# mxngjxa/lshrs

Measured on AMD Instinct MI355X. Metric: vectors/sec hashed (768-d, num_perm=256), higher is better.
Workload: dtype bf16x3 on the matrix cores + f32 replay of the host BLAS inside the proven window (bit-exact f32 sign result)

## Files before the change

lshrs_amd/csrc/sig_replay.hip:

```cpp
#include "lshrs_common.h"

using namespace lshrs;

namespace {
__device__ __forceinline__ void fix_chain_tile(const f32x4 (&p4)[2][4], const f32x4 (&x4)[2][4], float& acc, float& ss) {
#pragma unroll
  for (int sstep = 0; sstep < 16; ++sstep) {
    const int q = sstep >> 2, r = sstep & 3;
    acc = __builtin_fmaf(x4[0][q][r], p4[0][q][r], acc);
    acc = __builtin_fmaf(x4[1][q][r], p4[1][q][r], acc);
    ss = __builtin_fmaf(x4[0][q][r], x4[0][q][r], ss);
    ss = __builtin_fmaf(x4[1][q][r], x4[1][q][r], ss);
  }
}

__device__ __forceinline__ float blas_scalar_tail(float y, const float* __restrict__ pt, const float* __restrict__ xt, int m3,
                                                  int tail_model, bool count_ss, float* ss) {
  const float a0 = pt[0], x0 = xt[0];
  const float a1 = m3 > 1 ? pt[1] : 0.f, x1 = m3 > 1 ? xt[1] : 0.f;
  const float a2 = m3 > 2 ? pt[2] : 0.f, x2 = m3 > 2 ? xt[2] : 0.f;
  if (count_ss) *ss = __builtin_fmaf(x0, x0, __builtin_fmaf(x1, x1, __builtin_fmaf(x2, x2, *ss)));
  if (tail_model == 2) {
    float t = mul_then_add(0.f, a0, x0);
    if (m3 > 1) t = mul_then_add(t, a1, x1);
    if (m3 > 2) t = mul_then_add(t, a2, x2);
    return mul_then_add(y, t, 1.0f);
  }
  if (m3 == 1) return __builtin_fmaf(a0, x0, y);
  float t = __builtin_fmaf(a0, x0, mul_then_add(0.f, a1, x1));
  if (m3 > 2) t = __builtin_fmaf(a2, x2, t);
  return mul_then_add(y, t, 1.0f);
}

static_assert(LSHRS_SIG_COUNTERS + kFixParts * kFixGridG <= LSHRS_SIG_DEVICE_COUNTERS, "stage 2's per-workgroup slots must fit the counter block");
template <bool REPLAY, bool GENERAL = false, int SLAB = kFixSlabG, bool SAMEP = false>
__global__ __launch_bounds__(64) void sig_fix8_kernel(const FixArgs a) {
  static_assert(!SAMEP || (REPLAY && SLAB * 8 <= 64), "the shared hyperplane slab is one LDS-DMA of the wave");
  __shared__ __attribute__((aligned(16))) f32x4 xs[2][SLAB * 8 * kFixG];
  __shared__ __attribute__((aligned(16))) f32x4 ps[2][SAMEP ? 64 : SLAB * 8 * kFixG];
  const int lane = threadIdx.x, g = lane & (kFixG - 1), sub = lane >> 3;
  const int shh = sub >> 2, sq = sub & 3;
  const int64_t* __restrict__ list = SAMEP ? a.sorted_list : a.flag_list;
  const float* __restrict__ ylist = SAMEP ? a.sorted_y : a.flag_y;
  __shared__ int gstart[SAMEP ? kSortMaxCols + 1 : 1];
  const bool buckets = SAMEP && a.col_cap > 0;
  if (SAMEP && buckets) {
    constexpr int kPer = kSortMaxCols / 64;
    int mine[kPer], sum = 0;
    bool over = false;
#pragma unroll
    for (int i = 0; i < kPer; ++i) {
      const int c = lane * kPer + i;
      const int want = c < a.padcols ? a.col_count[c] : 0;
      over = over || want > a.col_cap;
      mine[i] = ((want < a.col_cap ? want : a.col_cap) + kFixG - 1) / kFixG;
      sum += mine[i];
    }
    int incl = sum;
#pragma unroll
    for (int off = 1; off < 64; off <<= 1) {
      const int v = __shfl_up(incl, off);
      if (lane >= off) incl += v;
    }
    int at = incl - sum;
#pragma unroll
    for (int i = 0; i < kPer; ++i) {
      gstart[lane * kPer + i] = at;
      at += mine[i];
    }
    if (lane == 63) gstart[kSortMaxCols] = at;
    if (blockIdx.x == 0 && __any(over) && lane == 0) *a.overflow = 1;
    __syncthreads();
  }
  const int cnt = !SAMEP ? min(*a.flag_count, a.flag_cap) : gstart[kSortMaxCols] * kFixG;
  const int fgroups = (cnt + kFixG - 1) / kFixG;
  const int groups = fgroups + (!SAMEP && REPLAY && a.audit_list != nullptr ? (a.audit_n + kFixG - 1) / kFixG : 0);
  const size_t ldp = (size_t)a.ktiles * kKTile;
  const int head = GENERAL ? (a.dim & 4) : 0;
  const int m3 = GENERAL ? (a.dim & 3) : 0;
  const int body = GENERAL ? a.dim - m3 - head : a.ktiles * kKTile;
  const int kt = GENERAL ? (body + kKTile - 1) / kKTile : a.ktiles;
  const int slabs = (kt + SLAB - 1) / SLAB;
  int n_ties = 0, n_flips = 0, n_aud = 0, n_abad = 0;
  float max_dev = 0.f, max_ratio = 0.f;
  struct Item { int64_t row; int col; bool live; const float* xg; const float* pg; const float* xrow; int e; bool audit; };
  auto fetch = [&](int grp) {
    Item it;
    it.audit = grp >= fgroups;
    int64_t item;
    bool inlist;
    if (SAMEP && buckets) {
      int lo = 0, hi = a.padcols - 1;
      while (lo < hi) {
        const int mid = (lo + hi + 1) >> 1;
        if (gstart[mid] <= grp) lo = mid; else hi = mid - 1;
      }
      const int off = (grp - gstart[lo]) * kFixG + g;
      const int have = min(a.col_count[lo], a.col_cap);
      inlist = off < have;
      it.e = lo * a.col_cap + (inlist ? off : 0);
      item = list[it.e];
      it.audit = (item & kAuditBit) != 0;
      item &= ~kAuditBit;
    } else if (!it.audit) {
      it.e = grp * kFixG + g;
      inlist = it.e < cnt;
      item = list[inlist ? it.e : grp * kFixG];
    } else {
      it.e = (grp - fgroups) * kFixG + g;
      item = it.e < a.audit_n ? a.audit_list[it.e] : -1;
      inlist = item >= 0;
      if (!inlist) item = 0;
    }
    it.row = entry_row(item);
    const int col_raw = entry_col(item);
    it.live = inlist && col_raw < a.padcols;
    it.col = col_raw < a.padcols ? col_raw : 0;
    it.xrow = a.X + it.row * a.ldx;
    it.xg = it.xrow + head + 16 * shh + 4 * sq;
    it.pg = a.prow + (size_t)it.col * ldp + head + 16 * shh + 4 * sq;
#ifdef LSHRS_AB_FIX_SAME_P
    {
      const int c0 = entry_col(a.flag_list[grp * kFixG < cnt ? grp * kFixG : 0]);
      it.pg = a.prow + (size_t)(c0 < a.padcols ? c0 : 0) * ldp + 16 * shh + 4 * sq;
    }
#endif
    return it;
  };
  auto issue = [&](const Item& it, int slab, int buf) {
#pragma unroll
    for (int i = 0; i < SLAB; ++i) {
      const int t = slab * SLAB + i < kt ? slab * SLAB + i : kt - 1;
#ifndef LSHRS_AB_FIX_NO_X
      const float* xsrc = it.xg + (size_t)t * kKTile;
      if (GENERAL && t * kKTile + 16 * shh + 4 * sq >= body) xsrc = it.xrow;
      __builtin_amdgcn_global_load_lds((const GLOBAL_AS void*)xsrc, (LDS_AS void*)(xs[buf] + i * 64), 16, 0, 0);
#endif
#ifndef LSHRS_AB_FIX_NO_P
      if (!SAMEP)
        __builtin_amdgcn_global_load_lds((const GLOBAL_AS void*)(it.pg + (size_t)t * kKTile), (LDS_AS void*)(ps[buf] + i * 64),
                                         16, 0, 0);
#endif
    }
    if (SAMEP) {
      const int ti = (lane >> 3) < SLAB ? (lane >> 3) : SLAB - 1;
      const int t = slab * SLAB + ti < kt ? slab * SLAB + ti : kt - 1;
      const float* psrc = a.prow + (size_t)it.col * ldp + head + (size_t)t * kKTile + 4 * (lane & 7);
      __builtin_amdgcn_global_load_lds((const GLOBAL_AS void*)psrc, (LDS_AS void*)ps[buf], 16, 0, 0);
    }
  };
  int grp = blockIdx.x;
  if (grp < groups) {
  Item cur = fetch(grp);
  issue(cur, 0, 0);
  int buf = 0;
  for (;;) {
    const int nxt_grp = grp + (int)gridDim.x;
    const bool has_next = nxt_grp < groups;
    Item nxt = cur;
    if (has_next) nxt = fetch(nxt_grp);
    const int64_t row = cur.row;
    const int col = cur.col, e = cur.e;
    const bool live = cur.live;
    const int word = col >> 5, c = col & 31;
    float acc = 0.f, ss = 0.f, pj = 0.f, ytot = 0.f;
    bool blocks_done = false;
    const int kind = GENERAL ? blas_row_kind(col % a.band_cols, a.rows_per_band) : 0;
    if (GENERAL && head != 0) {
      const int hl = kind == 1 ? (sub & 3) : sub;
      if (hl < 4) {
        const float hx = cur.xrow[hl];
        pj = a.prow[(size_t)col * ldp + hl] * hx;
        if (sub < 4) ss = hx * hx;
      }
    }
    for (int sl = 0; sl < slabs; ++sl) {
      const int tiles = kt - sl * SLAB < SLAB ? kt - sl * SLAB : SLAB;
      bool more = true;
      if (sl + 1 < slabs) issue(cur, sl + 1, buf ^ 1);
      else if (has_next) issue(nxt, 0, buf ^ 1);
      else more = false;
#if defined(LSHRS_AB_FIX_NO_X) || defined(LSHRS_AB_FIX_NO_P)
      if (more) wait_vmcnt<SLAB>();
#else
      if (more) wait_vmcnt<SAMEP ? SLAB + 1 : 2 * SLAB>();
#endif
      else asm volatile("s_waitcnt vmcnt(0)" ::: "memory");
      if (REPLAY) {
        const float* xf = reinterpret_cast<const float*>(xs[buf]);
        const float* pf = reinterpret_cast<const float*>(ps[buf]);
        if (!GENERAL) {
#pragma unroll 3
          for (int t = 0; t < tiles; ++t) {
#pragma unroll
            for (int m = 0; m < 4; ++m) {
              const int o = ((t * 8 + 2 * m + (sub >> 2)) * kFixG + g) * 4 + (sub & 3);
              const int op = SAMEP ? (t * 8 + 2 * m + (sub >> 2)) * 4 + (sub & 3) : o;
              const float xv = xf[o];
              pj = __builtin_fmaf(pf[op], xv, pj);
              ss = __builtin_fmaf(xv, xv, ss);
            }
          }
        } else {
          for (int t = 0; t < tiles; ++t) {
            const int kb0 = (sl * SLAB + t) * kKTile;
#pragma unroll
            for (int m = 0; m < 4; ++m) {
              const int o = ((t * 8 + 2 * m + (sub >> 2)) * kFixG + g) * 4 + (sub & 3);
              const int op = SAMEP ? (t * 8 + 2 * m + (sub >> 2)) * 4 + (sub & 3) : o;
              const bool in = kb0 + 8 * m + sub < body;
              const float xv = in ? xf[o] : 0.f, pv = in ? pf[op] : 0.f;
              ss = __builtin_fmaf(xv, xv, ss);
              if (kind == 1) {
                const int o0 = ((t * 8 + 2 * m) * kFixG + g) * 4 + (sub & 3), o1 = o0 + kFixG * 4;
                const int p0 = SAMEP ? (t * 8 + 2 * m) * 4 + (sub & 3) : o0, p1 = SAMEP ? p0 + 4 : o1;
                const int kl = kb0 + 8 * m + (sub & 3);
                pj = mul_then_add(pj, kl < body ? pf[p0] : 0.f, kl < body ? xf[o0] : 0.f);
                pj = mul_then_add(pj, kl + 4 < body ? pf[p1] : 0.f, kl + 4 < body ? xf[o1] : 0.f);
              } else if (kind == 2) {
                pj = mul_then_add(pj, pv, xv);
              } else {
                pj = __builtin_fmaf(pv, xv, pj);
              }
            }
            const int tile = sl * SLAB + t + 1;
            if ((tile % kBlasBlockTiles) == 0 && tile < kt) {
              const float sblk = blas_reduce(pj, kind, lane);
              ytot = blocks_done ? ytot + sblk : sblk;
              blocks_done = true;
              pj = 0.f;
            }
          }
        }
      } else {
#pragma unroll 2
        for (int t = 0; t < tiles; ++t) {
          f32x4 p4[2][4], x4[2][4];
#pragma unroll
          for (int hh = 0; hh < 2; ++hh)
#pragma unroll
            for (int q = 0; q < 4; ++q) {
              x4[hh][q] = xs[buf][(t * 8 + hh * 4 + q) * kFixG + g];
              p4[hh][q] = ps[buf][(t * 8 + hh * 4 + q) * kFixG + g];
            }
          fix_chain_tile(p4, x4, acc, ss);
        }
      }
      asm volatile("s_waitcnt lgkmcnt(0)" ::: "memory");
      buf ^= 1;
    }
    float yb = 0.f;
    if (REPLAY) {
      yb = blas_reduce(pj, kind, lane);
      if (GENERAL && blocks_done) yb = ytot + yb;
      if (GENERAL && m3 != 0)
        yb = blas_scalar_tail(yb, a.prow + (size_t)col * ldp + head + body, cur.xrow + head + body, m3, a.tail_model, sub == 0, &ss);
      float s2 = ss + __shfl(ss, (lane + 32) & 63);
      s2 += __shfl(s2, (lane + 8) & 63);
      ss = s2 + __shfl(s2, (lane + 16) & 63);
    }
    if (REPLAY && cur.audit) {
      if (sub == 0 && live) {
        const uint8_t kbyte = a.keys[row * (int64_t)a.row_bytes + (col >> 3)];
        ++n_aud;
        if ((yb > 0.f) != (((kbyte >> (col & 7)) & 1) != 0)) ++n_abad;
        const float y1 = (SAMEP && buckets) ? ylist[e] : a.audit_vals[2 * e];
        const float thr = (SAMEP && buckets) ? a.flag_thr[e] : a.audit_vals[2 * e + 1];
        if (thr > 0.f) {
          const float ratio = __builtin_fabsf(y1 - yb) / thr;
          if (ratio < __builtin_inff()) max_ratio = __builtin_fmaxf(max_ratio, ratio);
        }
      }
    } else if (sub == 0 && live) {
    uint8_t* kb = a.keys + row * (int64_t)a.row_bytes + (col >> 3);
    const uintptr_t addr = reinterpret_cast<uintptr_t>(kb);
    unsigned int* w32 = reinterpret_cast<unsigned int*>(addr & ~(uintptr_t)3);
    const unsigned int bitmask = 1u << (8 * (unsigned)(addr & 3) + (col & 7));
    bool want = acc > 0.f;
    const bool have = (*kb >> (col & 7)) & 1;
    if (REPLAY) {
      want = yb > 0.f;
      const float scale = sqrtf(ss) * a.norms[col];
      if (__builtin_fabsf(yb) < a.tau * sqrtf(ss) * a.tie_coef[col]) ++n_ties;
      if (want != have) ++n_flips;
      if (ylist != nullptr && scale > 0.f) {
        const float dev = __builtin_fabsf(ylist[e] - yb) / (scale * 0x1p-24f);
        if (dev < __builtin_inff()) max_dev = __builtin_fmaxf(max_dev, dev);
      }
    }
    if (want != have) {
      if (want) atomicOr(w32, bitmask);
      else atomicAnd(w32, ~bitmask);
    }
    if (!REPLAY && a.tie_list != nullptr) {
      const float thr = a.tau * sqrtf(ss) * a.tie_coef[col];
      if (__builtin_fabsf(acc) < thr) {
        const int slot = atomicAdd(a.tie_count, 1);
        if (slot < a.tie_cap) {
          a.tie_list[2 * (int64_t)slot] = (row + a.row_base) * 65536 + word;
          a.tie_list[2 * (int64_t)slot + 1] = (int64_t)(1u << c);
        }
      }
    }
    if (REPLAY && a.replay_y != nullptr) a.replay_y[e] = yb;
    }
    if (!has_next) break;
    cur = nxt;
    grp = nxt_grp;
  }
  }
  if (REPLAY) {
#pragma unroll
    for (int off = 1; off < 8; off <<= 1) {
      n_ties += __shfl_xor(n_ties, off);
      n_flips += __shfl_xor(n_flips, off);
      max_dev = __builtin_fmaxf(max_dev, __shfl_xor(max_dev, off));
      n_aud += __shfl_xor(n_aud, off);
      n_abad += __shfl_xor(n_abad, off);
      max_ratio = __builtin_fmaxf(max_ratio, __shfl_xor(max_ratio, off));
    }
    if (lane == 0) {
      int* p = a.partials + kFixParts * blockIdx.x;
      p[0] = a.count_ties ? n_ties : 0;
      p[1] = n_flips;
      p[2] = __float_as_int(max_dev);
      p[3] = n_aud;
      p[4] = n_abad;
      p[5] = __float_as_int(max_ratio);
    }
  }
}

__global__ void expand_ties_kernel(const int64_t* __restrict__ tie_list, const int* __restrict__ tie_count, int tie_cap,
                                   int padcols, int64_t* __restrict__ flag_list, int flag_cap, int* flag_count) {
  const int cnt = min(*tie_count, tie_cap);
  for (int e = blockIdx.x * blockDim.x + threadIdx.x; e < cnt; e += gridDim.x * blockDim.x) {
    const int64_t row = tie_list[2 * (int64_t)e] >> 16;
    const int word = (int)(tie_list[2 * (int64_t)e] & 0xFFFF);
    unsigned mask = (unsigned)tie_list[2 * (int64_t)e + 1];
    const int m = __popc(mask);
    if (m == 0) continue;
    int slot = atomicAdd(flag_count, m);
    while (mask != 0u) {
      const int c = __ffs(mask) - 1;
      mask &= mask - 1u;
      const int col = 32 * word + c;
      if (slot < flag_cap && col < padcols) flag_list[slot] = flag_entry(row, col);
      else if (slot < flag_cap) flag_list[slot] = flag_entry(row, (1 << kEntryColBits) - 1);
      ++slot;
    }
  }
}

__device__ __forceinline__ float mul_rounded(float a, float b) {
#pragma clang fp contract(off)
  return a * b;
}
__device__ __forceinline__ float add_rounded(float a, float b) {
#pragma clang fp contract(off)
  return a + b;
}
__device__ __forceinline__ float small_skx_dot(const float* __restrict__ a, const float* __restrict__ x, int n, int row, int rows) {
  auto p = [&](int k) { return mul_rounded(a[k], x[k]); };
  auto f = [&](int k, float s) { return __builtin_fmaf(a[k], x[k], s); };
  const int b16 = rows / 16 * 16, b8 = rows / 8 * 8;
  int rem = rows - b8, type;
  if (row < b16) type = 16;
  else if (row < b8) type = 8;
  else if (rem >= 4 && row < b8 + 4) type = 4;
  else {
    const int base = b8 + (rem >= 4 ? 4 : 0);
    rem -= rem >= 4 ? 4 : 0;
    type = (rem >= 2 && row < base + 2) ? 2 : 1;
  }
  auto seq = [&]() {
    float s = p(0);
    for (int k = 1; k < n; ++k) s = add_rounded(s, p(k));
    return s;
  };
  auto chain = [&]() {
    float s = p(0);
    for (int k = 1; k < n; ++k) s = f(k, s);
    return s;
  };
  switch (n) {
    case 1: return p(0);
    case 2: return type == 16 ? f(1, p(0)) : add_rounded(p(0), p(1));
    case 3:
      if (type >= 8) return f(2, f(1, p(0)));
      if (type == 2) return add_rounded(add_rounded(p(0), p(1)), p(2));
      return f(2, f(0, p(1)));
    case 4: return type == 1 ? seq() : add_rounded(add_rounded(p(0), p(1)), add_rounded(p(2), p(3)));
    case 5: return type >= 4 ? chain() : seq();
    case 6:
      if (type >= 8) return chain();
      if (type == 4) return add_rounded(add_rounded(p(0), f(1, p(2))), add_rounded(p(3), f(4, p(5))));
      return seq();
    case 7:
      if (type >= 8) return chain();
      if (type == 4) return add_rounded(add_rounded(f(0, p(1)), f(4, p(5))), add_rounded(f(2, p(3)), p(6)));
      return seq();
    default:
      if (type >= 4)
        return add_rounded(add_rounded(add_rounded(p(0), p(1)), add_rounded(p(2), p(3))), add_rounded(add_rounded(p(4), p(5)), add_rounded(p(6), p(7))));
      if (type == 2)
        return add_rounded(add_rounded(add_rounded(p(0), p(1)), add_rounded(p(4), p(5))), add_rounded(add_rounded(p(2), p(3)), add_rounded(p(6), p(7))));
      return add_rounded(add_rounded(add_rounded(add_rounded(p(0), p(4)), add_rounded(p(1), p(5))), add_rounded(p(2), p(6))), add_rounded(p(3), p(7)));
  }
}

__global__ __launch_bounds__(64) void sig_fixany_kernel(const FixArgs a) {
  const int lane = threadIdx.x, g = lane & (kFixG - 1), sub = lane >> 3;
  const int cnt = min(*a.flag_count, a.flag_cap);
  const int fgroups = (cnt + kFixG - 1) / kFixG;
  const int groups = fgroups + (a.audit_list != nullptr ? (a.audit_n + kFixG - 1) / kFixG : 0);
  const size_t ldp = (size_t)a.ktiles * kKTile;
  const int body = a.dim & ~3, m3 = a.dim & 3;
  int n_ties = 0, n_flips = 0, n_aud = 0, n_abad = 0;
  float max_dev = 0.f, max_ratio = 0.f;
  for (int grp = blockIdx.x; grp < groups; grp += gridDim.x) {
    const bool audit = grp >= fgroups;
    const int e = (audit ? grp - fgroups : grp) * kFixG + g;
    int64_t item;
    bool inlist;
    if (!audit) {
      inlist = e < cnt;
      item = a.flag_list[inlist ? e : grp * kFixG];
    } else {
      item = e < a.audit_n ? a.audit_list[e] : -1;
      inlist = item >= 0;
      if (!inlist) item = 0;
    }
    const int64_t row = entry_row(item);
    const int col_raw = entry_col(item);
    const bool live = inlist && col_raw < a.padcols;
    const int col = col_raw < a.padcols ? col_raw : 0;
    const float* __restrict__ xr = a.X + row * a.ldx;
    const float* __restrict__ pr = a.prow + (size_t)col * ldp;
    const int kind = blas_row_kind(col % a.band_cols, a.rows_per_band);
    float y = 0.f, ss = 0.f;
    if (a.tail_model == 3) {
      const int j = col % a.band_cols;
      y = j < a.rows_per_band ? small_skx_dot(pr, xr, a.dim, j, a.rows_per_band) : 0.f;
      if (sub == 0)
        for (int k = 0; k < a.dim; ++k) ss = __builtin_fmaf(xr[k], xr[k], ss);
    } else if (a.rows_per_band == 1) {
      const int n1 = a.dim & ~31;
      float kernel = 0.f;
      if (a.tail_model == 1) {
        const int n64 = n1 & ~63;
        float acc[8] = {0.f, 0.f, 0.f, 0.f, 0.f, 0.f, 0.f, 0.f};
        for (int k0 = 0; k0 < n64; k0 += 64)
#pragma unroll
          for (int j = 0; j < 8; ++j) {
            const float xv = xr[k0 + 8 * j + sub];
            acc[j] = __builtin_fmaf(pr[k0 + 8 * j + sub], xv, acc[j]);
            ss = __builtin_fmaf(xv, xv, ss);
          }
        float t[4];
#pragma unroll
        for (int u = 0; u < 4; ++u) t[u] = n64 > 0 ? acc[2 * u] + acc[2 * u + 1] : 0.f;
        if (n64 < n1) {
#pragma unroll
          for (int u = 0; u < 4; ++u) {
            const float xv = xr[n64 + 8 * u + sub];
            t[u] = __builtin_fmaf(pr[n64 + 8 * u + sub], xv, t[u]);
            ss = __builtin_fmaf(xv, xv, ss);
          }
        }
        const float v = ((t[0] + t[1]) + t[2]) + t[3];
        kernel = blas_reduce(v, 0, lane);
      } else {
        float acc[4] = {0.f, 0.f, 0.f, 0.f};
        for (int k0 = 0; k0 < n1; k0 += 32)
#pragma unroll
          for (int j = 0; j < 4; ++j) {
            const float xv = xr[k0 + 8 * j + sub];
            acc[j] = __builtin_fmaf(pr[k0 + 8 * j + sub], xv, acc[j]);
            ss = __builtin_fmaf(xv, xv, ss);
          }
        float sj[4];
#pragma unroll
// ... 23 lines not shown
      } else {
        const int head = kn & 4;
        if (head != 0 && sub < 4) {
          const float xv = xr[k0 + sub];
          pj = pr[k0 + sub] * xv;
          ss = __builtin_fmaf(xv, xv, ss);
        }
        for (int k = k0 + head + sub; k < k0 + kn; k += 8) {
          const float xv = xr[k];
          pj = kind == 0 ? __builtin_fmaf(pr[k], xv, pj) : mul_then_add(pj, pr[k], xv);
          ss = __builtin_fmaf(xv, xv, ss);
        }
      }
      const float sblk = blas_reduce(pj, kind, lane);
      y = k0 == 0 ? sblk : y + sblk;
    }
    if (m3 != 0 && a.rows_per_band != 1 && a.tail_model != 3)
      y = blas_scalar_tail(y, pr + body, xr + body, m3, a.tail_model, sub == 0, &ss);
    float s2 = ss + __shfl(ss, (lane + 32) & 63);
    s2 += __shfl(s2, (lane + 8) & 63);
    s2 += __shfl(s2, (lane + 16) & 63);
    if (sub == 0 && live && audit) {
      const uint8_t kbyte = a.keys[row * (int64_t)a.row_bytes + (col >> 3)];
      ++n_aud;
      if ((y > 0.f) != (((kbyte >> (col & 7)) & 1) != 0)) ++n_abad;
      const float thr = a.audit_vals[2 * e + 1];
      if (thr > 0.f) {
        const float ratio = __builtin_fabsf(a.audit_vals[2 * e] - y) / thr;
        if (ratio < __builtin_inff()) max_ratio = __builtin_fmaxf(max_ratio, ratio);
      }
    } else if (sub == 0 && live) {
      uint8_t* kb = a.keys + row * (int64_t)a.row_bytes + (col >> 3);
      const uintptr_t addr = reinterpret_cast<uintptr_t>(kb);
      unsigned int* w32 = reinterpret_cast<unsigned int*>(addr & ~(uintptr_t)3);
      const unsigned int bitmask = 1u << (8 * (unsigned)(addr & 3) + (col & 7));
      const bool want = y > 0.f;
      const bool have = (*kb >> (col & 7)) & 1;
      if (__builtin_fabsf(y) < a.tau * sqrtf(s2) * a.tie_coef[col]) ++n_ties;
      if (a.flag_y != nullptr) {
        const float scale = sqrtf(s2) * a.norms[col];
        if (scale > 0.f) {
          const float dev = __builtin_fabsf(a.flag_y[e] - y) / (scale * 0x1p-24f);
          if (dev < __builtin_inff()) max_dev = __builtin_fmaxf(max_dev, dev);
        }
      }
      if (want != have) {
        ++n_flips;
        if (want) atomicOr(w32, bitmask);
        else atomicAnd(w32, ~bitmask);
      }
      if (a.replay_y != nullptr) a.replay_y[e] = y;
    }
  }
#pragma unroll
  for (int off = 1; off < 8; off <<= 1) {
    n_ties += __shfl_xor(n_ties, off);
    n_flips += __shfl_xor(n_flips, off);
    max_dev = __builtin_fmaxf(max_dev, __shfl_xor(max_dev, off));
    n_aud += __shfl_xor(n_aud, off);
    n_abad += __shfl_xor(n_abad, off);
    max_ratio = __builtin_fmaxf(max_ratio, __shfl_xor(max_ratio, off));
  }
  if (lane == 0) {
    int* p = a.partials + kFixParts * blockIdx.x;
    p[0] = a.count_ties ? n_ties : 0;
    p[1] = n_flips;
    p[2] = __float_as_int(max_dev);
    p[3] = n_aud;
    p[4] = n_abad;
    p[5] = __float_as_int(max_ratio);
  }
}

constexpr int kExportThreads = 1024;
__global__ __launch_bounds__(kExportThreads) void export_counts_kernel(int* counters, int* host_counts, int nparts, int* zero = nullptr,
                                                                      int nzero = 0, int* done = nullptr, int epoch = 0) {
  __shared__ int fold[kExportThreads / 64][kFixParts];
  const int tid = threadIdx.x, lane = tid & 63, wave = tid >> 6;
  for (int i = tid; i < nzero; i += kExportThreads) zero[i] = 0;
  int* parts = counters + LSHRS_SIG_COUNTERS;
  int ties = 0, flips = 0, dev = 0, aud = 0, abad = 0, ratio = 0;
  for (int i = tid; i < nparts; i += kExportThreads) {
    int* q = parts + kFixParts * i;
    ties += q[0];
    flips += q[1];
    dev = max(dev, q[2]);
    aud += q[3];
    abad += q[4];
    ratio = max(ratio, q[5]);
    q[0] = q[1] = q[2] = q[3] = q[4] = q[5] = 0;
  }
#pragma unroll
  for (int off = 32; off >= 1; off >>= 1) {
    ties += __shfl_xor(ties, off);
    flips += __shfl_xor(flips, off);
    dev = max(dev, __shfl_xor(dev, off));
    aud += __shfl_xor(aud, off);
    abad += __shfl_xor(abad, off);
    ratio = max(ratio, __shfl_xor(ratio, off));
  }
  if (lane == 0) {
    fold[wave][0] = ties; fold[wave][1] = flips; fold[wave][2] = dev;
    fold[wave][3] = aud; fold[wave][4] = abad; fold[wave][5] = ratio;
  }
  __syncthreads();
  if (tid < LSHRS_SIG_COUNTERS) {
    ties = flips = dev = aud = abad = ratio = 0;
    for (int w = 0; w < kExportThreads / 64; ++w) {
      ties += fold[w][0];
      flips += fold[w][1];
      dev = max(dev, fold[w][2]);
      aud += fold[w][3];
      abad += fold[w][4];
      ratio = max(ratio, fold[w][5]);
    }
    int v = counters[tid];
    if (tid == 0) v += ties;
    if (tid == 2) v = max(v, dev);
    if (tid == 3) v += flips;
    if (tid == 4) v += aud;
    if (tid == 5) v += abad;
    if (tid == 6) v = max(v, ratio);
    if (host_counts != nullptr) {
      host_counts[tid] = v;
      counters[tid] = 0;
    } else {
      counters[tid] = v;
    }
  }
  if (done != nullptr) {
    __threadfence_system();
    __syncthreads();
    if (tid == 0) {
      __hip_atomic_store(done, epoch, __ATOMIC_RELEASE, __HIP_MEMORY_SCOPE_SYSTEM);
    }
  }
}
}

uint32_t lshrs_flags_replay(void) {
  uint32_t f = 0;
#ifdef LSHRS_AB_FIX_SAME_P
  f |= LSHRS_BUILD_WRONG_KEYS | (1u << 8);
#endif
#ifdef LSHRS_AB_FIX_NO_X
  f |= LSHRS_BUILD_WRONG_KEYS | (1u << 9);
#endif
#ifdef LSHRS_AB_FIX_NO_P
  f |= LSHRS_BUILD_WRONG_KEYS | (1u << 10);
#endif
#if LSHRS_FIX_SLAB != 6 || LSHRS_FIX_GRID != 1536
  f |= LSHRS_BUILD_TUNED | (1u << 21);
#endif
#if defined(LSHRS_BUCKET_GRID) || defined(LSHRS_BUCKET_SLAB)
  f |= LSHRS_BUILD_TUNED | (1u << 22);
#endif
  return f;
}

template <int SLAB, bool SAMEP>
static void launch_replay(bool general, dim3 grid, const FixArgs& f, hipStream_t s, hipEvent_t start, hipEvent_t stop) {
  dispatch_bool(general, [&](auto gen) {
    hipExtLaunchKernelGGL((sig_fix8_kernel<true, decltype(gen)::value, SLAB, SAMEP>), grid, dim3(64), 0, s, start, stop, 0, f);
  });
}

int lshrs_replay_stage2(const FixArgs& f, int32_t* counters, int32_t* host_counts, const Opts& o, hipStream_t s) {
  const int blas_model = f.blas_model, rows_per_band = f.rows_per_band, dim = f.dim, flag_cap = f.flag_cap;
  const int64_t* flag_list = f.flag_list;
  const float* flag_y = f.flag_y;
  const int* flag_count = f.flag_count;
  const bool general = blas_general(rows_per_band, f.ktiles, dim);
  const int64_t groups = ((int64_t)flag_cap + kFixG - 1) / kFixG;
  const bool short_rows = f.ktiles <= kFixSlabShort && blas_model != 0;
  const int grid_cap = short_rows ? kFixGridShort : kFixGridG;
  const dim3 grid((unsigned)(groups < grid_cap ? groups : grid_cap)), block(64);
  if (blas_model != 0) {
    int nparts = (int)grid.x;
    if (rows_per_band == 1) {
      const int64_t agroups = f.audit_list != nullptr ? ((int64_t)f.audit_n + kFixG - 1) / kFixG : 0;
      const int64_t want = groups + agroups;
      const dim3 ogrid((unsigned)(want < kFixGridG ? want : kFixGridG));
      hipExtLaunchKernelGGL(sig_fixany_kernel, ogrid, block, 0, s, o.ev[2], o.ev[3], 0, f);
      nparts = (int)ogrid.x;
    } else if (short_rows) {
      launch_replay<kFixSlabShort, false>(general, grid, f, s, o.ev[2], o.ev[3]);
    } else if (f.col_cap > 0) {
#ifndef LSHRS_BUCKET_GRID
#define LSHRS_BUCKET_GRID 2048
#endif
#ifndef LSHRS_BUCKET_SLAB
#define LSHRS_BUCKET_SLAB LSHRS_FIX_SLAB
#endif
      constexpr int kBucketGrid = LSHRS_BUCKET_GRID, kBucketSlab = LSHRS_BUCKET_SLAB;
      const int64_t bgroups = (int64_t)f.padcols * ((f.col_cap + kFixG - 1) / kFixG);
      const dim3 bgrid((unsigned)(bgroups < kBucketGrid ? bgroups : kBucketGrid));
      FixArgs fb = f;
      fb.audit_list = nullptr;
      fb.audit_n = 0;
      fb.overflow = counters + 7;
      launch_replay<kBucketSlab, true>(general, bgrid, fb, s, o.ev[2], o.ev[3]);
      hipLaunchKernelGGL(export_counts_kernel, dim3(1), dim3(kExportThreads), 0, s, counters, host_counts, (int)bgrid.x,
                         o.sort->hist + (size_t)(1 - (o.sort->parity & 1)) * kSortMaxCols, kSortMaxCols, o.done, o.epoch);
      return -(int)hipGetLastError();
    } else {
      launch_replay<kFixSlabG, false>(general, grid, f, s, o.ev[2], o.ev[3]);
    }
    hipLaunchKernelGGL(export_counts_kernel, dim3(1), dim3(kExportThreads), 0, s, counters, host_counts, nparts, nullptr, 0, o.done,
                       o.epoch);
  } else {
    hipExtLaunchKernelGGL((sig_fix8_kernel<false, false>), grid, block, 0, s, o.ev[2], o.ev[3], 0, f);
  }
  return -(int)hipGetLastError();
}

struct TiesPlan { SigGeom g; int row_bytes; bool plain; };
static int ties_replay_plan(const float* X, int64_t n, int64_t ldx, const void* workspace, int32_t num_bands, int32_t rows_per_band, int32_t dim,
                            const uint8_t* keys, bool lists_ok, int32_t blas_model, TiesPlan* p) {
  if (X == nullptr || workspace == nullptr || keys == nullptr || !lists_ok || n < 0 || ldx < dim ||
      !sig_shape_ok(num_bands, rows_per_band, dim) || (blas_model != 1 && blas_model != 2 && blas_model != 3) ||
      (blas_model == 3 && (dim > 8 || rows_per_band < 2)))
    return LSHRS_E_BADARG;
  const SigGeom g = sig_geom(num_bands, rows_per_band, dim);
  const bool fast = dim % 4 == 0 && dim >= 8 && ldx % 4 == 0 && (reinterpret_cast<uintptr_t>(X) & 15) == 0 && rows_per_band >= 2 &&
                    blas_model != 3;
  const int body = dim & ~3;
  const bool one_row = rows_per_band == 1;
  if (!one_row && dim < 9 && dim % 4 != 0 && blas_model == 1) return LSHRS_E_TOOLARGE;
  const bool short_last_block = body % 8 != 0 && body > 4096;
  if (n >= ((int64_t)1 << 42) || (fast && !short_last_block && blas_model != 1)) return LSHRS_E_TOOLARGE;
  *p = TiesPlan{g, num_bands * g.bb, !fast || short_last_block};
  return 0;
}

static void ties_replay_launch(FixArgs& f, const TiesPlan& p, int32_t* counters, int32_t* host_counts, hipStream_t s) {
  f.partials = counters + LSHRS_SIG_COUNTERS;
  const int64_t groups = ((int64_t)f.flag_cap + kFixG - 1) / kFixG;
  const dim3 grid((unsigned)(groups < kFixGridG ? groups : kFixGridG)), block(64);
  f.tail_model = f.blas_model;
  if (p.plain) hipLaunchKernelGGL(sig_fixany_kernel, grid, block, 0, s, f);
  else launch_replay<kFixSlabG, false>(blas_general(f.rows_per_band, p.g.ktiles, f.dim), grid, f, s, nullptr, nullptr);
  hipLaunchKernelGGL(export_counts_kernel, dim3(1), dim3(kExportThreads), 0, s, counters, host_counts, (int)grid.x);
}

extern "C" {

int lshrs_sig_resolve_ties_replay_f32(const float* X, int64_t n, int64_t ldx, const void* workspace, int32_t num_bands,
                                       int32_t rows_per_band, int32_t dim, uint8_t* keys, const int64_t* tie_list,
                                       int32_t tie_cap, int32_t* counters, float tau, int64_t* flag_list,
                                       int32_t flag_cap, int32_t blas_model, int32_t* host_counts, void* stream) {
  int32_t* tie_count = counters;
  int32_t* flag_count = counters != nullptr ? counters + 1 : nullptr;
  if (n == 0) return 0;
  TiesPlan p;
  const int rc = ties_replay_plan(X, n, ldx, workspace, num_bands, rows_per_band, dim, keys,
                                  tie_list != nullptr && tie_count != nullptr && flag_list != nullptr && tie_cap > 0 && flag_cap > 0,
                                  blas_model, &p);
  if (rc != 0) return rc;
  hipStream_t s = static_cast<hipStream_t>(stream);
  const float* base = static_cast<const float*>(workspace);
  {
    const int threads = 256;
    const int blocks = tie_cap < 256 * 64 ? (tie_cap + threads - 1) / threads : 64;
    hipLaunchKernelGGL(expand_ties_kernel, dim3((unsigned)blocks), dim3(threads), 0, s, tie_list, tie_count, tie_cap,
                       p.row_bytes * 8, flag_list, flag_cap, flag_count);
  }
  FixArgs f = fix_args_base(X, ldx, dim, base, p.g, rows_per_band, keys, p.row_bytes, flag_list, flag_count, flag_cap, tau, blas_model);
  ties_replay_launch(f, p, counters, host_counts, s);
  return -(int)hipGetLastError();
}

int lshrs_sig_replay_values_f32(const float* X, int64_t n, int64_t ldx, const void* workspace, int32_t num_bands,
                                int32_t rows_per_band, int32_t dim, int32_t blas_model, int32_t route, uint8_t* keys,
                                float* values, int64_t* list, int32_t list_cap, const lshrs_sig_sort* sort,
                                int32_t* counters, void* stream) {
  if (n == 0) return 0;
  if (values == nullptr || counters == nullptr) return LSHRS_E_BADARG;
  constexpr float kValuesTau = 8 * 0x1p-24f;
  hipStream_t s = static_cast<hipStream_t>(stream);
  if (route == LSHRS_REPLAY_ROUTE_SMALL) {
    if (list != nullptr || sort != nullptr) return LSHRS_E_BADARG;
    return lshrs_small_replay(X, n, ldx, workspace, num_bands, rows_per_band, dim, keys, nullptr, counters, kValuesTau, blas_model,
                              nullptr, 0, values, stream);
  }
  if (route == LSHRS_REPLAY_ROUTE_TIES) {
    TiesPlan p;
    const int rc = ties_replay_plan(X, n, ldx, workspace, num_bands, rows_per_band, dim, keys, list != nullptr && list_cap > 0 && sort == nullptr,
                                    blas_model, &p);
    if (rc != 0) return rc;
    FixArgs f = fix_args_base(X, ldx, dim, static_cast<const float*>(workspace), p.g, rows_per_band, keys, p.row_bytes, list, counters + 1,
                              list_cap, kValuesTau, blas_model);
    f.replay_y = values;
    ties_replay_launch(f, p, counters, nullptr, s);
    return -(int)hipGetLastError();
  }
  if (route != LSHRS_REPLAY_ROUTE_STAGE2) return LSHRS_E_BADARG;
  Opts o;
  if (sort != nullptr) {
    if (list != nullptr || sort->struct_bytes < sizeof(lshrs_sig_sort) || sort->list == nullptr || sort->y == nullptr || sort->hist == nullptr ||
        sort->cap <= 0)
      return LSHRS_E_BADARG;
    o.sort = sort;
  }
  FixArgs f;
  const int rc = lshrs_split_stage2_args(X, n, ldx, workspace, num_bands, rows_per_band, dim, keys, counters, kValuesTau,
                                         sort != nullptr ? sort->list : list, nullptr, sort != nullptr ? sort->cap : list_cap, blas_model, o,
                                         sort != nullptr, &f);
  if (rc != 0) return rc;
  f.replay_y = values;
  return lshrs_replay_stage2(f, counters, nullptr, o, s);
}

}
```

Before: 853.1 million.

## Restructure bucketed replay into contiguous column runs with LDS-resident hyperplane row

The sorted-bucket (same-hyperplane) replay path moves into a new fix8_columns routine. Each workgroup now takes a contiguous range of groups instead of a grid-stride with a per-group binary search. The hyperplane row for the current column is kept resident in dynamic LDS and reloaded only when the column changes. Entry, y, threshold and key bytes are staged through LDS-DMA, tiles are read with hand-written ds_read asm, and a configurable 2- or 3-deep ring is used. The grid is sized to the occupancy the LDS budget allows, which trades more code complexity and heavier LDS use for fewer global loads of the hyperplane and less per-item scheduling overhead.

```diff
diff --git a/lshrs_amd/csrc/sig_replay.hip b/lshrs_amd/csrc/sig_replay.hip
--- a/lshrs_amd/csrc/sig_replay.hip
+++ b/lshrs_amd/csrc/sig_replay.hip
@@ -33,48 +33,367 @@
 }
 
 static_assert(LSHRS_SIG_COUNTERS + kFixParts * kFixGridG <= LSHRS_SIG_DEVICE_COUNTERS, "stage 2's per-workgroup slots must fit the counter block");
+
+__device__ __forceinline__ void fix_store_stats(const FixArgs& a, int lane, int n_ties, int n_flips, float max_dev, int n_aud, int n_abad,
+                                                float max_ratio) {
+#pragma unroll
+  for (int off = 1; off < 8; off <<= 1) {
+    n_ties += __shfl_xor(n_ties, off);
+    n_flips += __shfl_xor(n_flips, off);
+    max_dev = __builtin_fmaxf(max_dev, __shfl_xor(max_dev, off));
+    n_aud += __shfl_xor(n_aud, off);
+    n_abad += __shfl_xor(n_abad, off);
+    max_ratio = __builtin_fmaxf(max_ratio, __shfl_xor(max_ratio, off));
+  }
+  if (lane == 0) {
+    int* p = a.partials + kFixParts * blockIdx.x;
+    p[0] = a.count_ties ? n_ties : 0;
+    p[1] = n_flips;
+    p[2] = __float_as_int(max_dev);
+    p[3] = n_aud;
+    p[4] = n_abad;
+    p[5] = __float_as_int(max_ratio);
+  }
+}
+
+__device__ __forceinline__ unsigned lds_offset(const void* p) { return (unsigned)reinterpret_cast<uintptr_t>((LDS_AS const void*)p); }
+__device__ __forceinline__ unsigned lds_read_b32(unsigned at) {
+  unsigned v;
+  asm volatile("ds_read_b32 %0, %1\n\ts_waitcnt lgkmcnt(0)" : "=v"(v) : "v"(at) : "memory");
+  return v;
+}
+__device__ __forceinline__ void lds_read_b64(unsigned at, unsigned& lo, unsigned& hi) {
+  asm volatile("ds_read_b32 %0, %2\n\tds_read_b32 %1, %2 offset:4\n\ts_waitcnt lgkmcnt(0)" : "=&v"(lo), "=&v"(hi) : "v"(at) : "memory");
+}
+__device__ __forceinline__ void lds_read_tile(unsigned xat, unsigned pat, float (&x)[4], float (&p)[4]) {
+  asm volatile(
+      "ds_read_b32 %0, %8\n\tds_read_b32 %4, %9\n\t"
+      "ds_read_b32 %1, %8 offset:256\n\tds_read_b32 %5, %9 offset:32\n\t"
+      "ds_read_b32 %2, %8 offset:512\n\tds_read_b32 %6, %9 offset:64\n\t"
+      "ds_read_b32 %3, %8 offset:768\n\tds_read_b32 %7, %9 offset:96\n\t"
+      "s_waitcnt lgkmcnt(0)"
+      : "=&v"(x[0]), "=&v"(x[1]), "=&v"(x[2]), "=&v"(x[3]), "=&v"(p[0]), "=&v"(p[1]), "=&v"(p[2]), "=&v"(p[3])
+      : "v"(xat), "v"(pat)
+      : "memory");
+}
+__device__ __forceinline__ int scalar_load_b32(const void* p) {
+  int v;
+  asm volatile("s_load_dword %0, %1, 0x0\n\ts_waitcnt lgkmcnt(0)" : "=s"(v) : "s"(p) : "memory");
+  return v;
+}
+
+constexpr int kFixResidentTiles = kBlasBlockTiles;
+#ifndef LSHRS_BUCKET_RING
+#define LSHRS_BUCKET_RING 2
+#endif
+__host__ __device__ inline int fix_body_tiles(bool general, int dim, int ktiles) {
+  return general ? ((dim & ~3) - (dim & 4) + kKTile - 1) / kKTile : ktiles;
+}
+inline size_t fix_columns_lds(bool general, int dim, int ktiles) {
+  const int kt = fix_body_tiles(general, dim, ktiles);
+  return kt <= kFixResidentTiles ? (size_t)kt * 128 : (size_t)LSHRS_BUCKET_RING * 1024;
+}
+inline int fix_columns_per_cu(int slab, size_t row_lds) {
+  return (int)((size_t)160 * 1024 / ((size_t)LSHRS_BUCKET_RING * slab * 1024 + 1024 + row_lds));
+}
+
+template <bool GENERAL, int SLAB>
+__device__ __forceinline__ void fix8_columns(const FixArgs& a) {
+  constexpr int NB = LSHRS_BUCKET_RING;
+  static_assert(NB == 2 || NB == 3, "one slab read, one or two landing");
+  __shared__ __attribute__((aligned(16))) f32x4 xs[NB][SLAB * 8 * kFixG];
+  __shared__ __attribute__((aligned(16))) unsigned stage[2][2][64];
+  extern __shared__ __attribute__((aligned(16))) f32x4 prow_lds[];
+  const int lane = threadIdx.x, g = lane & (kFixG - 1), sub = lane >> 3;
+  const int shh = sub >> 2, sq = sub & 3;
+  const int64_t* __restrict__ list = a.sorted_list;
+  const float* __restrict__ ylist = a.sorted_y;
+  const size_t ldp = (size_t)a.ktiles * kKTile;
+  const int head = GENERAL ? (a.dim & 4) : 0;
+  const int m3 = GENERAL ? (a.dim & 3) : 0;
+  const int body = GENERAL ? a.dim - m3 - head : a.ktiles * kKTile;
+  const int kt = fix_body_tiles(GENERAL, a.dim, a.ktiles);
+  const int slabs = (kt + SLAB - 1) / SLAB;
+  const bool resident = !GENERAL || kt <= kFixResidentTiles;
+  const int ahead = (NB == 3 && slabs >= 2) ? 2 : 1;
+  int n_ties = 0, n_flips = 0, n_aud = 0, n_abad = 0;
+  float max_dev = 0.f, max_ratio = 0.f;
+
+  constexpr int kPer = kSortMaxCols / 64;
+  int mine[kPer], sum = 0;
+  bool over = false;
+#pragma unroll
+  for (int i = 0; i < kPer; ++i) {
+    const int c = lane * kPer + i;
+    const int want = c < a.padcols ? a.col_count[c] : 0;
+    over = over || want > a.col_cap;
+    mine[i] = ((want < a.col_cap ? want : a.col_cap) + kFixG - 1) / kFixG;
+    sum += mine[i];
+  }
+  int incl = sum;
+#pragma unroll
+  for (int off = 1; off < 64; off <<= 1) {
+    const int v = __shfl_up(incl, off);
+    if (lane >= off) incl += v;
+  }
+  const int at = incl - sum;
+  const int total = __builtin_amdgcn_readlane(incl, 63);
+  if (blockIdx.x == 0 && __any(over) && lane == 0) *a.overflow = 1;
+  const int first = (int)((int64_t)blockIdx.x * total / (int)gridDim.x);
+  int left = (int)(((int64_t)blockIdx.x + 1) * total / (int)gridDim.x) - first;
+  if (left > 0) {
+  const int owner = 63 - __builtin_clzll(__ballot(at <= first));
+  int c_own = 0, o_own = 0;
+  {
+    int s = at;
+#pragma unroll
+    for (int i = 0; i < kPer; ++i) {
+      if (first >= s && first < s + mine[i]) {
+        c_own = lane * kPer + i;
+        o_own = first - s;
+      }
+      s += mine[i];
+    }
+  }
+  struct Pos { int col, off, cnt; float norm, coef; };
+  auto enter = [&](int c, int off) {
+    int cnt;
+    for (;;) {
+      const int want = scalar_load_b32(a.col_count + c);
+      cnt = want < a.col_cap ? want : a.col_cap;
+      if (cnt > 0 || c + 1 >= a.padcols) break;
+      ++c;
+    }
+    return Pos{c, off, cnt, __int_as_float(scalar_load_b32(a.norms + c)), __int_as_float(scalar_load_b32(a.tie_coef + c))};
+  };
+  auto advance = [&](const Pos& p) {
+    if ((p.off + 1) * kFixG < p.cnt) return Pos{p.col, p.off + 1, p.cnt, p.norm, p.coef};
+    return enter(p.col + 1, 0);
+  };
+  const unsigned stage_at = lds_offset(stage), xs_at = lds_offset(xs), prow_at = lds_offset(prow_lds);
+  auto stage_entries = [&](const Pos& p, int par) {
+    const int l5 = lane & 31, j = l5 < 16 ? l5 >> 1 : l5 & 7;
+    const int o = p.off * kFixG + j;
+    const size_t e = (size_t)p.col * a.col_cap + (o < p.cnt ? o : 0);
+    const unsigned* src = reinterpret_cast<const unsigned*>(list + e) + (l5 & 1);
+    if (l5 >= 16 && l5 < 24 && ylist != nullptr) src = reinterpret_cast<const unsigned*>(ylist + e);
+    if (l5 >= 24 && a.flag_thr != nullptr) src = reinterpret_cast<const unsigned*>(a.flag_thr + e);
+    __builtin_amdgcn_global_load_lds((const GLOBAL_AS void*)src, (LDS_AS void*)stage[par][0], 4, 0, 0);
+  };
+  struct Item { int64_t row; bool live, audit; int e; const float* xrow; const float* xg; uintptr_t kaddr; };
+  auto resolve = [&](const Pos& p, int par) {
+    Item it;
+    unsigned lo, hi;
+    lds_read_b64(stage_at + (unsigned)par * 512u + 8u * (unsigned)g, lo, hi);
+    int64_t item = (int64_t)(((uint64_t)hi << 32) | lo);
+    it.audit = (item & kAuditBit) != 0;
+    item &= ~kAuditBit;
+    it.row = entry_row(item);
+    const int o = p.off * kFixG + g;
+    const bool inlist = o < p.cnt;
+    it.e = p.col * a.col_cap + (inlist ? o : 0);
+    it.live = inlist && entry_col(item) < a.padcols;
+    it.xrow = a.X + it.row * a.ldx;
+    it.xg = it.xrow + head + 16 * shh + 4 * sq;
+    it.kaddr = reinterpret_cast<uintptr_t>(a.keys + it.row * (int64_t)a.row_bytes + (p.col >> 3));
+    __builtin_amdgcn_global_load_lds((const GLOBAL_AS void*)(it.kaddr & ~(uintptr_t)3), (LDS_AS void*)stage[par][1], 4, 0, 0);
+    return it;
+  };
+  auto row_part = [&](int col, int t0, int n) {
+#ifndef LSHRS_AB_FIX_NO_P
+    if ((lane >> 3) < n) {
+      const float* psrc = a.prow + (size_t)col * ldp + head + (size_t)(t0 + (lane >> 3)) * kKTile + 4 * (lane & 7);
+      __builtin_amdgcn_global_load_lds((const GLOBAL_AS void*)psrc, (LDS_AS void*)(prow_lds + t0 * 8), 16, 0, 0);
+    }
+#endif
+  };
+  auto issue = [&](const Item& it, int col, int slab, int buf) {
+#ifndef LSHRS_AB_FIX_NO_X
+#pragma unroll
+    for (int i = 0; i < SLAB; ++i) {
+      const int t = slab * SLAB + i < kt ? slab * SLAB + i : kt - 1;
+      const float* xsrc = it.xg + (size_t)t * kKTile;
+      if (GENERAL && t * kKTile + 16 * shh + 4 * sq >= body) xsrc = it.xrow;
+      __builtin_amdgcn_global_load_lds((const GLOBAL_AS void*)xsrc, (LDS_AS void*)(xs[buf] + i * 64), 16, 0, 0);
+    }
+#endif
+    if (GENERAL && !resident) {
+      const int ti = (lane >> 3) < SLAB ? (lane >> 3) : SLAB - 1;
+      const int t = slab * SLAB + ti < kt ? slab * SLAB + ti : kt - 1;
+      const float* psrc = a.prow + (size_t)col * ldp + head + (size_t)t * kKTile + 4 * (lane & 7);
+      __builtin_amdgcn_global_load_lds((const GLOBAL_AS void*)psrc, (LDS_AS void*)(prow_lds + buf * 64), 16, 0, 0);
+    }
+  };
+  auto wait_ring = [&](bool more) {
+#if defined(LSHRS_AB_FIX_NO_X)
+    asm volatile("s_waitcnt vmcnt(0)" ::: "memory");
+#else
+    if (!more) asm volatile("s_waitcnt vmcnt(0)" ::: "memory");
+    else if (GENERAL && !resident) { if (ahead == 2) wait_vmcnt<2 * (SLAB + 1)>(); else wait_vmcnt<SLAB + 1>(); }
+    else if (ahead == 2) wait_vmcnt<2 * SLAB>();
+    else wait_vmcnt<SLAB>();
+#endif
+  };
+
+  Pos pc = enter(__builtin_amdgcn_readlane(c_own, owner), __builtin_amdgcn_readlane(o_own, owner));
+  int par = 0, buf = 0;
+  stage_entries(pc, 0);
+  asm volatile("s_waitcnt vmcnt(0)" ::: "memory");
+  Item cur = resolve(pc, 0);
+  if (resident)
+    for (int t0 = 0; t0 < kt; t0 += 8) row_part(pc.col, t0, kt - t0 < 8 ? kt - t0 : 8);
+  issue(cur, pc.col, 0, 0);
+  if (ahead == 2) issue(cur, pc.col, 1, 1);
+  for (;;) {
+    const bool has_next = left > 1;
+    Pos pn = pc;
+    Item nxt = cur;
+    if (has_next) {
+      pn = advance(pc);
+      stage_entries(pn, par ^ 1);
+    }
+    const bool turn = resident && has_next && pn.col != pc.col;
+    const int64_t row = cur.row;
+    const int col = pc.col, e = cur.e;
+    const bool live = cur.live;
+    float ss = 0.f, pj = 0.f, ytot = 0.f;
+    bool blocks_done = false;
+    const int kind = GENERAL ? blas_row_kind(col % a.band_cols, a.rows_per_band) : 0;
+    if (GENERAL && head != 0) {
+      const int hl = kind == 1 ? (sub & 3) : sub;
+      if (hl < 4) {
+        const float hx = cur.xrow[hl];
+        pj = a.prow[(size_t)col * ldp + hl] * hx;
+        if (sub < 4) ss = hx * hx;
+      }
+    }
+    for (int sl = 0; sl < slabs; ++sl) {
+      const int tiles = kt - sl * SLAB < SLAB ? kt - sl * SLAB : SLAB;
+      const int is = sl + ahead, ibuf = (buf + ahead) % NB;
+      bool more = true;
+      if (is < slabs) {
+        issue(cur, col, is, ibuf);
+      } else if (has_next) {
+        if (is == slabs) {
+          if (slabs < 2 * ahead) asm volatile("s_waitcnt vmcnt(0)" ::: "memory");
+          nxt = resolve(pn, par ^ 1);
+        }
+        issue(nxt, pn.col, is - slabs, ibuf);
+      } else {
+        more = false;
+      }
+      wait_ring(more);
+      const unsigned pslab = prow_at + (resident ? (unsigned)(sl * SLAB) * 128u : (unsigned)buf * 1024u);
+      const unsigned xslab = xs_at + (unsigned)buf * (SLAB * 1024u);
+      if (!GENERAL) {
+        unsigned xat = xslab + (((sub >> 2) * kFixG + g) * 4 + (sub & 3)) * 4u, pat = pslab + ((sub >> 2) * 4 + (sub & 3)) * 4u;
+        for (int t = 0; t < tiles; ++t, xat += 1024u, pat += 128u) {
+          float xv[4], pv[4];
+          lds_read_tile(xat, pat, xv, pv);
+#pragma unroll
+          for (int m = 0; m < 4; ++m) {
+            pj = __builtin_fmaf(pv[m], xv[m], pj);
+            ss = __builtin_fmaf(xv[m], xv[m], ss);
+          }
+        }
+      } else {
+        unsigned xat = xslab + (g * 4 + (sub & 3)) * 4u, pat = pslab + (sub & 3) * 4u;
+        for (int t = 0; t < tiles; ++t, xat += 1024u, pat += 128u) {
+          const int kb0 = (sl * SLAB + t) * kKTile;
+          float x0[4], p0[4], x1[4], p1[4];
+          lds_read_tile(xat, pat, x0, p0);
+          lds_read_tile(xat + 128u, pat + 16u, x1, p1);
+#pragma unroll
+          for (int m = 0; m < 4; ++m) {
+            const bool in = kb0 + 8 * m + sub < body;
+            const float xv = in ? ((sub >> 2) ? x1[m] : x0[m]) : 0.f, pv = in ? ((sub >> 2) ? p1[m] : p0[m]) : 0.f;
+            ss = __builtin_fmaf(xv, xv, ss);
+            if (kind == 1) {
+              const int kl = kb0 + 8 * m + (sub & 3);
+              pj = mul_then_add(pj, kl < body ? p0[m] : 0.f, kl < body ? x0[m] : 0.f);
+              pj = mul_then_add(pj, kl + 4 < body ? p1[m] : 0.f, kl + 4 < body ? x1[m] : 0.f);
+            } else if (kind == 2) {
+              pj = mul_then_add(pj, pv, xv);
+            } else {
+              pj = __builtin_fmaf(pv, xv, pj);
+            }
+          }
+          const int tile = sl * SLAB + t + 1;
+          if ((tile % kBlasBlockTiles) == 0 && tile < kt) {
+            const float sblk = blas_reduce(pj, kind, lane);
+            ytot = blocks_done ? ytot + sblk : sblk;
+            blocks_done = true;
+            pj = 0.f;
+          }
+        }
+      }
+      asm volatile("s_waitcnt lgkmcnt(0)" ::: "memory");
+      if (turn) row_part(pn.col, sl * SLAB, tiles);
+      buf = buf + 1 == NB ? 0 : buf + 1;
+    }
+    float yb = blas_reduce(pj, kind, lane);
+    if (GENERAL && blocks_done) yb = ytot + yb;
+    if (GENERAL && m3 != 0)
+      yb = blas_scalar_tail(yb, a.prow + (size_t)col * ldp + head + body, cur.xrow + head + body, m3, a.tail_model, sub == 0, &ss);
+    float s2 = ss + __shfl(ss, (lane + 32) & 63);
+    s2 += __shfl(s2, (lane + 8) & 63);
+    ss = s2 + __shfl(s2, (lane + 16) & 63);
+    const unsigned mine_at = stage_at + (unsigned)par * 512u;
+    const float y1 = __uint_as_float(lds_read_b32(mine_at + (16u + g) * 4u));
+    const float thr = __uint_as_float(lds_read_b32(mine_at + (24u + g) * 4u));
+    const unsigned kbyte = (lds_read_b32(mine_at + 256u + g * 4u) >> (8 * (unsigned)(cur.kaddr & 3))) & 0xFFu;
+    const bool have = (kbyte >> (col & 7)) & 1;
+    if (cur.audit) {
+      if (sub == 0 && live) {
+        ++n_aud;
+        if ((yb > 0.f) != have) ++n_abad;
+        if (thr > 0.f) {
+          const float ratio = __builtin_fabsf(y1 - yb) / thr;
+          if (ratio < __builtin_inff()) max_ratio = __builtin_fmaxf(max_ratio, ratio);
+        }
+      }
+    } else if (sub == 0 && live) {
+      GLOBAL_AS unsigned int* w32 = (GLOBAL_AS unsigned int*)(cur.kaddr & ~(uintptr_t)3);
+      const unsigned int bitmask = 1u << (8 * (unsigned)(cur.kaddr & 3) + (col & 7));
+      const bool want = yb > 0.f;
+      const float scale = sqrtf(ss) * pc.norm;
+      if (__builtin_fabsf(yb) < a.tau * sqrtf(ss) * pc.coef) ++n_ties;
+      if (want != have) ++n_flips;
+      if (ylist != nullptr && scale > 0.f) {
+        const float dev = __builtin_fabsf(y1 - yb) / (scale * 0x1p-24f);
+        if (dev < __builtin_inff()) max_dev = __builtin_fmaxf(max_dev, dev);
+      }
+      if (want != have) {
+        if (want) __hip_atomic_fetch_or(w32, bitmask, __ATOMIC_RELAXED, __HIP_MEMORY_SCOPE_AGENT);
+        else __hip_atomic_fetch_and(w32, ~bitmask, __ATOMIC_RELAXED, __HIP_MEMORY_SCOPE_AGENT);
+      }
+      if (a.replay_y != nullptr) a.replay_y[e] = yb;
+    }
+    if (!has_next) break;
+    cur = nxt;
+    pc = pn;
+    par ^= 1;
+    --left;
+  }
+  }
+  fix_store_stats(a, lane, n_ties, n_flips, max_dev, n_aud, n_abad, max_ratio);
+}
+
 template <bool REPLAY, bool GENERAL = false, int SLAB = kFixSlabG, bool SAMEP = false>
 __global__ __launch_bounds__(64) void sig_fix8_kernel(const FixArgs a) {
-  static_assert(!SAMEP || (REPLAY && SLAB * 8 <= 64), "the shared hyperplane slab is one LDS-DMA of the wave");
+  static_assert(!SAMEP || (REPLAY && SLAB <= 8), "a slab of the shared hyperplane row is one LDS-DMA of the wave");
+  if constexpr (SAMEP) {
+    fix8_columns<GENERAL, SLAB>(a);
+  } else {
   __shared__ __attribute__((aligned(16))) f32x4 xs[2][SLAB * 8 * kFixG];
-  __shared__ __attribute__((aligned(16))) f32x4 ps[2][SAMEP ? 64 : SLAB * 8 * kFixG];
+  __shared__ __attribute__((aligned(16))) f32x4 ps[2][SLAB * 8 * kFixG];
   const int lane = threadIdx.x, g = lane & (kFixG - 1), sub = lane >> 3;
   const int shh = sub >> 2, sq = sub & 3;
-  const int64_t* __restrict__ list = SAMEP ? a.sorted_list : a.flag_list;
-  const float* __restrict__ ylist = SAMEP ? a.sorted_y : a.flag_y;
-  __shared__ int gstart[SAMEP ? kSortMaxCols + 1 : 1];
-  const bool buckets = SAMEP && a.col_cap > 0;
-  if (SAMEP && buckets) {
-    constexpr int kPer = kSortMaxCols / 64;
-    int mine[kPer], sum = 0;
-    bool over = false;
-#pragma unroll
-    for (int i = 0; i < kPer; ++i) {
-      const int c = lane * kPer + i;
-      const int want = c < a.padcols ? a.col_count[c] : 0;
-      over = over || want > a.col_cap;
-      mine[i] = ((want < a.col_cap ? want : a.col_cap) + kFixG - 1) / kFixG;
-      sum += mine[i];
-    }
-    int incl = sum;
-#pragma unroll
-    for (int off = 1; off < 64; off <<= 1) {
-      const int v = __shfl_up(incl, off);
-      if (lane >= off) incl += v;
-    }
-    int at = incl - sum;
-#pragma unroll
-    for (int i = 0; i < kPer; ++i) {
-      gstart[lane * kPer + i] = at;
-      at += mine[i];
-    }
-    if (lane == 63) gstart[kSortMaxCols] = at;
-    if (blockIdx.x == 0 && __any(over) && lane == 0) *a.overflow = 1;
-    __syncthreads();
-  }
-  const int cnt = !SAMEP ? min(*a.flag_count, a.flag_cap) : gstart[kSortMaxCols] * kFixG;
+  const int64_t* __restrict__ list = a.flag_list;
+  const float* __restrict__ ylist = a.flag_y;
+  const int cnt = min(*a.flag_count, a.flag_cap);
   const int fgroups = (cnt + kFixG - 1) / kFixG;
-  const int groups = fgroups + (!SAMEP && REPLAY && a.audit_list != nullptr ? (a.audit_n + kFixG - 1) / kFixG : 0);
+  const int groups = fgroups + (REPLAY && a.audit_list != nullptr ? (a.audit_n + kFixG - 1) / kFixG : 0);
   const size_t ldp = (size_t)a.ktiles * kKTile;
   const int head = GENERAL ? (a.dim & 4) : 0;
   const int m3 = GENERAL ? (a.dim & 3) : 0;
@@ -89,20 +408,7 @@
     it.audit = grp >= fgroups;
     int64_t item;
     bool inlist;
-    if (SAMEP && buckets) {
-      int lo = 0, hi = a.padcols - 1;
-      while (lo < hi) {
-        const int mid = (lo + hi + 1) >> 1;
-        if (gstart[mid] <= grp) lo = mid; else hi = mid - 1;
-      }
-      const int off = (grp - gstart[lo]) * kFixG + g;
-      const int have = min(a.col_count[lo], a.col_cap);
-      inlist = off < have;
-      it.e = lo * a.col_cap + (inlist ? off : 0);
-      item = list[it.e];
-      it.audit = (item & kAuditBit) != 0;
-      item &= ~kAuditBit;
-    } else if (!it.audit) {
+    if (!it.audit) {
       it.e = grp * kFixG + g;
       inlist = it.e < cnt;
       item = list[inlist ? it.e : grp * kFixG];
@@ -137,16 +443,8 @@
       __builtin_amdgcn_global_load_lds((const GLOBAL_AS void*)xsrc, (LDS_AS void*)(xs[buf] + i * 64), 16, 0, 0);
 #endif
 #ifndef LSHRS_AB_FIX_NO_P
-      if (!SAMEP)
-        __builtin_amdgcn_global_load_lds((const GLOBAL_AS void*)(it.pg + (size_t)t * kKTile), (LDS_AS void*)(ps[buf] + i * 64),
-                                         16, 0, 0);
-#endif
-    }
-    if (SAMEP) {
-      const int ti = (lane >> 3) < SLAB ? (lane >> 3) : SLAB - 1;
-      const int t = slab * SLAB + ti < kt ? slab * SLAB + ti : kt - 1;
-      const float* psrc = a.prow + (size_t)it.col * ldp + head + (size_t)t * kKTile + 4 * (lane & 7);
-      __builtin_amdgcn_global_load_lds((const GLOBAL_AS void*)psrc, (LDS_AS void*)ps[buf], 16, 0, 0);
+      __builtin_amdgcn_global_load_lds((const GLOBAL_AS void*)(it.pg + (size_t)t * kKTile), (LDS_AS void*)(ps[buf] + i * 64), 16, 0, 0);
+#endif
     }
   };
   int grp = blockIdx.x;
@@ -183,7 +481,7 @@
 #if defined(LSHRS_AB_FIX_NO_X) || defined(LSHRS_AB_FIX_NO_P)
       if (more) wait_vmcnt<SLAB>();
 #else
-      if (more) wait_vmcnt<SAMEP ? SLAB + 1 : 2 * SLAB>();
+      if (more) wait_vmcnt<2 * SLAB>();
 #endif
       else asm volatile("s_waitcnt vmcnt(0)" ::: "memory");
       if (REPLAY) {
@@ -195,9 +493,8 @@
 #pragma unroll
             for (int m = 0; m < 4; ++m) {
               const int o = ((t * 8 + 2 * m + (sub >> 2)) * kFixG + g) * 4 + (sub & 3);
-              const int op = SAMEP ? (t * 8 + 2 * m + (sub >> 2)) * 4 + (sub & 3) : o;
               const float xv = xf[o];
-              pj = __builtin_fmaf(pf[op], xv, pj);
+              pj = __builtin_fmaf(pf[o], xv, pj);
               ss = __builtin_fmaf(xv, xv, ss);
             }
           }
@@ -207,16 +504,14 @@
 #pragma unroll
             for (int m = 0; m < 4; ++m) {
               const int o = ((t * 8 + 2 * m + (sub >> 2)) * kFixG + g) * 4 + (sub & 3);
-              const int op = SAMEP ? (t * 8 + 2 * m + (sub >> 2)) * 4 + (sub & 3) : o;
               const bool in = kb0 + 8 * m + sub < body;
-              const float xv = in ? xf[o] : 0.f, pv = in ? pf[op] : 0.f;
+              const float xv = in ? xf[o] : 0.f, pv = in ? pf[o] : 0.f;
               ss = __builtin_fmaf(xv, xv, ss);
               if (kind == 1) {
                 const int o0 = ((t * 8 + 2 * m) * kFixG + g) * 4 + (sub & 3), o1 = o0 + kFixG * 4;
-                const int p0 = SAMEP ? (t * 8 + 2 * m) * 4 + (sub & 3) : o0, p1 = SAMEP ? p0 + 4 : o1;
                 const int kl = kb0 + 8 * m + (sub & 3);
-                pj = mul_then_add(pj, kl < body ? pf[p0] : 0.f, kl < body ? xf[o0] : 0.f);
-                pj = mul_then_add(pj, kl + 4 < body ? pf[p1] : 0.f, kl + 4 < body ? xf[o1] : 0.f);
+                pj = mul_then_add(pj, kl < body ? pf[o0] : 0.f, kl < body ? xf[o0] : 0.f);
+                pj = mul_then_add(pj, kl + 4 < body ? pf[o1] : 0.f, kl + 4 < body ? xf[o1] : 0.f);
               } else if (kind == 2) {
                 pj = mul_then_add(pj, pv, xv);
               } else {
@@ -264,8 +559,7 @@
         const uint8_t kbyte = a.keys[row * (int64_t)a.row_bytes + (col >> 3)];
         ++n_aud;
         if ((yb > 0.f) != (((kbyte >> (col & 7)) & 1) != 0)) ++n_abad;
-        const float y1 = (SAMEP && buckets) ? ylist[e] : a.audit_vals[2 * e];
-        const float thr = (SAMEP && buckets) ? a.flag_thr[e] : a.audit_vals[2 * e + 1];
+        const float y1 = a.audit_vals[2 * e], thr = a.audit_vals[2 * e + 1];
         if (thr > 0.f) {
           const float ratio = __builtin_fabsf(y1 - yb) / thr;
           if (ratio < __builtin_inff()) max_ratio = __builtin_fmaxf(max_ratio, ratio);
@@ -328,6 +622,7 @@
       p[4] = n_abad;
       p[5] = __float_as_int(max_ratio);
     }
+  }
   }
 }
 
@@ -657,16 +952,16 @@
 #if LSHRS_FIX_SLAB != 6 || LSHRS_FIX_GRID != 1536
   f |= LSHRS_BUILD_TUNED | (1u << 21);
 #endif
-#if defined(LSHRS_BUCKET_GRID) || defined(LSHRS_BUCKET_SLAB)
+#if defined(LSHRS_BUCKET_GRID) || defined(LSHRS_BUCKET_SLAB) || LSHRS_BUCKET_RING != 2
   f |= LSHRS_BUILD_TUNED | (1u << 22);
 #endif
   return f;
 }
 
 template <int SLAB, bool SAMEP>
-static void launch_replay(bool general, dim3 grid, const FixArgs& f, hipStream_t s, hipEvent_t start, hipEvent_t stop) {
+static void launch_replay(bool general, dim3 grid, const FixArgs& f, hipStream_t s, hipEvent_t start, hipEvent_t stop, size_t lds = 0) {
   dispatch_bool(general, [&](auto gen) {
-    hipExtLaunchKernelGGL((sig_fix8_kernel<true, decltype(gen)::value, SLAB, SAMEP>), grid, dim3(64), 0, s, start, stop, 0, f);
+    hipExtLaunchKernelGGL((sig_fix8_kernel<true, decltype(gen)::value, SLAB, SAMEP>), grid, dim3(64), lds, s, start, stop, 0, f);
   });
 }
 
@@ -692,19 +987,21 @@
       launch_replay<kFixSlabShort, false>(general, grid, f, s, o.ev[2], o.ev[3]);
     } else if (f.col_cap > 0) {
 #ifndef LSHRS_BUCKET_GRID
-#define LSHRS_BUCKET_GRID 2048
+#define LSHRS_BUCKET_GRID 1792
 #endif
 #ifndef LSHRS_BUCKET_SLAB
 #define LSHRS_BUCKET_SLAB LSHRS_FIX_SLAB
 #endif
       constexpr int kBucketGrid = LSHRS_BUCKET_GRID, kBucketSlab = LSHRS_BUCKET_SLAB;
+      const size_t row_lds = fix_columns_lds(general, dim, f.ktiles);
+      const int per_cu = fix_columns_per_cu(kBucketSlab, row_lds), resident = 256 * (per_cu < kBucketGrid / 256 ? per_cu : kBucketGrid / 256);
       const int64_t bgroups = (int64_t)f.padcols * ((f.col_cap + kFixG - 1) / kFixG);
-      const dim3 bgrid((unsigned)(bgroups < kBucketGrid ? bgroups : kBucketGrid));
+      const dim3 bgrid((unsigned)(bgroups < resident ? bgroups : resident));
       FixArgs fb = f;
       fb.audit_list = nullptr;
       fb.audit_n = 0;
       fb.overflow = counters + 7;
-      launch_replay<kBucketSlab, true>(general, bgrid, fb, s, o.ev[2], o.ev[3]);
+      launch_replay<kBucketSlab, true>(general, bgrid, fb, s, o.ev[2], o.ev[3], row_lds);
       hipLaunchKernelGGL(export_counts_kernel, dim3(1), dim3(kExportThreads), 0, s, counters, host_counts, (int)bgrid.x,
                          o.sort->hist + (size_t)(1 - (o.sort->parity & 1)) * kSortMaxCols, kSortMaxCols, o.done, o.epoch);
       return -(int)hipGetLastError();
```

Result: no change. 862.4 million, median of 6 (+1.1%).
